# dusk-network/dusk-blindbidproof

Hardware: AMD Instinct MI355X
Metric: blind-bid proofs/sec (higher is better)
Workload: dtype u32

## Files before the change

### dusk_blindbidproof_amd/csrc/msm.hip

```cpp
#include "context.h"

namespace bbp {

#ifndef BBP_FOLD_PRIO
#define BBP_FOLD_PRIO 2
#endif
#ifndef BBP_MSM_WAVES
#define BBP_MSM_WAVES 2
#endif
#ifndef BBP_MSM_WAVES_MAX
#define BBP_MSM_WAVES_MAX 2
#endif

#ifdef BBP_MSM_PROF
__device__ unsigned long long g_msm_prof[8];
#define MSM_PROF_BEGIN() unsigned long long prof_t = wall_clock64()
#define MSM_PROF_MARK(i)                                                    \
    if (tid == 0) {                                                         \
        unsigned long long now_ = wall_clock64();                           \
        atomicAdd(&g_msm_prof[i], now_ - prof_t);                           \
        prof_t = now_;                                                      \
    }
#else
#define MSM_PROF_BEGIN()
#define MSM_PROF_MARK(i)
#endif

__device__ __forceinline__ ge ge_shfl_down(const ge& p, int d) {
    ge r;
    const u32* w = reinterpret_cast<const u32*>(&p);
    u32* o = reinterpret_cast<u32*>(&r);
#pragma unroll
    for (int i = 0; i < GE_WORDS; i++) o[i] = (u32)__shfl_down((int)w[i], d, 64);
    return r;
}

__device__ __forceinline__ void xch_put(u32* xch, const ge& p) {
    const u32* w = reinterpret_cast<const u32*>(&p);
#pragma unroll
    for (int i = 0; i < GE_WORDS; i++) xch[i] = w[i];
}

__device__ __forceinline__ ge xch_get(const u32* xch) {
    ge p;
    u32* w = reinterpret_cast<u32*>(&p);
#pragma unroll
    for (int i = 0; i < GE_WORDS; i++) w[i] = xch[i];
    return p;
}

__device__ __forceinline__ row_regs load_row(const niels_row* __restrict__ tab, u32 entry, u32* __restrict__ fault) {
    u32 row = entry & 0x7fffffffu;
    if (row > (u32)(TAB_BASES * MSM_POS - 1)) {
        row = (u32)(TAB_BASES * MSM_POS - 1);
        atomicOr(fault, 1u);
    }
#ifdef BBP_EXP_ROWMASK
    row &= BBP_EXP_ROWMASK;
#endif
    return load_row_at(tab + row, entry >> 31);
}

#ifdef BBP_ACC_COOP
constexpr int COOP_IMG = 64 * 128;
__device__ __forceinline__ u32 coop_clamp_row(u32 entry, u32* __restrict__ fault) {
    u32 row = entry & 0x7fffffffu;
    if (row > (u32)(TAB_BASES * MSM_POS - 1)) {
        row = (u32)(TAB_BASES * MSM_POS - 1);
        atomicOr(fault, 1u);
    }
    return row;
}
__device__ __forceinline__ void coop_issue(const niels_row* __restrict__ tab, u8* wb, u32 my_row, int lane, u32 srcoff) {
    const u8* t = reinterpret_cast<const u8*>(tab);
    u32 r[8];
#pragma unroll
    for (int j = 0; j < 8; j++) r[j] = (u32)__shfl((int)my_row, 8 * j + (lane >> 3), 64);
#pragma unroll
    for (int j = 0; j < 8; j++) {
        const u8* src = t + (size_t)r[j] * 128 + (srcoff ^ (u32)((j & 1) << 6));
        __builtin_amdgcn_global_load_lds((const __attribute__((address_space(1))) void*)src, (__attribute__((address_space(3))) void*)(wb + j * 1024), 16, 0, 0);
    }
}
__device__ __forceinline__ row_regs coop_read(const u8* wb, u32 A, u32 neg) {
    const u32 An = A ^ (neg << 6);
    const uint4 a0 = *reinterpret_cast<const uint4*>(wb + An), a1 = *reinterpret_cast<const uint4*>(wb + (An ^ 0x10u));
    const uint2 a2 = *reinterpret_cast<const uint2*>(wb + (An ^ 0x20u));
    const uint4 b0 = *reinterpret_cast<const uint4*>(wb + (An ^ 0x40u)), b1 = *reinterpret_cast<const uint4*>(wb + (An ^ 0x50u));
    const uint2 b2 = *reinterpret_cast<const uint2*>(wb + (An ^ 0x60u));
    const uint2 x0 = *reinterpret_cast<const uint2*>(wb + (A ^ 0x20u) + 8);
    const uint4 x1 = *reinterpret_cast<const uint4*>(wb + (A ^ 0x30u));
    const uint2 x2 = *reinterpret_cast<const uint2*>(wb + (A ^ 0x60u) + 8), x3 = *reinterpret_cast<const uint2*>(wb + (A ^ 0x70u));
    row_regs r;
    r.ypx = fe{{(i32)a0.x, (i32)a0.y, (i32)a0.z, (i32)a0.w, (i32)a1.x, (i32)a1.y, (i32)a1.z, (i32)a1.w, (i32)a2.x, (i32)a2.y}};
    r.ymx = fe{{(i32)b0.x, (i32)b0.y, (i32)b0.z, (i32)b0.w, (i32)b1.x, (i32)b1.y, (i32)b1.z, (i32)b1.w, (i32)b2.x, (i32)b2.y}};
    r.xy2d = fe{{(i32)x0.x, (i32)x0.y, (i32)x1.x, (i32)x1.y, (i32)x1.z, (i32)x1.w, (i32)x2.x, (i32)x2.y, (i32)x3.x, (i32)x3.y}};
    return r;
}
#endif

__device__ __noinline__ void ge_add_nc(ge& r, const ge& a, const ge& b) { r = ge_add(a, b); }
__device__ __noinline__ void ge_dbl_nc(ge& r, const ge& a) { r = ge_dbl(a); }

#ifndef BBP_SORT_T
#define BBP_SORT_T 1024
#endif
constexpr int SORT_T = BBP_SORT_T;
template <int MODE> struct msm_geom;
template <> struct msm_geom<0> { static constexpr int K = MSM_K, NAF = MSM_NAF, W = MSM_W; };
template <> struct msm_geom<1> { static constexpr int K = FOLD_K, NAF = FOLD_NAF, W = FOLD_W; };
template <> struct msm_geom<2> { static constexpr int K = SMALL_K, NAF = SMALL_NAF, W = SMALL_W; };

template <int MODE>
__global__ __launch_bounds__(SORT_T) void k_msm_sort(const u32* __restrict__ scal_a, const u32* __restrict__ aux, u32 n_total, u32 n_idx_sets,
                                                      u32 n_sub, u32 split, u32* __restrict__ sorted_all, u32* __restrict__ cursor_all,
                                                      const u32* __restrict__ msm_map, const u32* __restrict__ n_active, u32* __restrict__ ticket) {
    constexpr int K = msm_geom<MODE>::K, NAF = msm_geom<MODE>::NAF, W = msm_geom<MODE>::W, G = K >= SORT_T ? K / SORT_T : 1;
    __shared__ u32 cursor[K + 1];
    __shared__ u32 part[SORT_T];
    const int tid = threadIdx.x;
    if (ticket && blockIdx.x == 0 && tid == 0) *ticket = 0;
    if (n_active && blockIdx.x >= *n_active) return;
    const size_t work = blockIdx.x, msm = work / split;
    const u32 i0 = (u32)(work % split) * n_sub;
    const u32 n = i0 < n_total ? min(n_sub, n_total - i0) : 0u;
    __builtin_amdgcn_s_setprio(3);
    const u32* sbase;
    const u32* base_idx = nullptr;
    u32 base0 = 0;
    if (MODE != 1) {
        const size_t src = msm_map ? (size_t)msm_map[msm] : msm;
        sbase = scal_a + (src * (size_t)n_total + i0) * 8;
        base_idx = aux + (size_t)(msm % n_idx_sets) * n_total + i0;
    } else {
        const u32 side = (u32)msm & 1u;
        sbase = (side ? aux : scal_a) + ((msm >> 1) * (size_t)2048 + i0) * 8;
        base0 = (side ? BBP_BASE_H0 : BBP_BASE_G0) + i0;
    }
    u32* sorted = sorted_all + work * (size_t)n_sub * W;
    auto key = [&](u32 i, u32 mag) -> u32 { return (MODE != 1 ? 0u : ((i0 + i) & (FOLD_CLS - 1)) * FOLD_M) + ((mag + 1) >> 1); };

    for (int k = tid; k <= K; k += SORT_T) cursor[k] = 0;
    __syncthreads();
    for (u32 i = tid; i < n; i += SORT_T) {
        const uint4* sp = reinterpret_cast<const uint4*>(sbase + (size_t)i * 8);
        uint4 lo = sp[0], hi = sp[1];
        const u32 s[8] = {lo.x, lo.y, lo.z, lo.w, hi.x, hi.y, hi.z, hi.w};
        if (MODE != 1 && base_idx[i] == MSM_SKIP_BASE) continue;
        sc_for_each_naf_digit<NAF>(s, [&](u32, u32 mag, u32) { atomicAdd(&cursor[key(i, mag)], 1u); });
    }
    __syncthreads();
    {
        u32 local = 0;
        for (int r = 1; r <= G; r++)
            if (tid * G + r <= K) local += cursor[tid * G + r];
        const int lane = tid & 63, wave = tid >> 6;
        u32 incl = local;
#pragma unroll
        for (int d = 1; d < 64; d <<= 1) {
            const u32 up = (u32)__shfl_up((int)incl, d, 64);
            if (lane >= d) incl += up;
        }
        if (lane == 63) part[wave] = incl;
        __syncthreads();
        if (tid < 64) {
            constexpr int NW = SORT_T / 64;
            u32 v = tid < NW ? part[tid] : 0u, sc_ = v;
#pragma unroll
            for (int d = 1; d < 64; d <<= 1) {
                const u32 up = (u32)__shfl_up((int)sc_, d, 64);
                if (tid >= d) sc_ += up;
            }
            if (tid < NW) part[tid] = sc_ - v;
        }
        __syncthreads();
        u32 base = part[wave] + incl - local;
        for (int r = 1; r <= G; r++) {
            if (tid * G + r > K) break;
            const u32 c = cursor[tid * G + r];
            cursor[tid * G + r] = base;
            base += c;
        }
    }
    __syncthreads();
    for (u32 i = tid; i < n; i += SORT_T) {
        const uint4* sp = reinterpret_cast<const uint4*>(sbase + (size_t)i * 8);
        uint4 lo = sp[0], hi = sp[1];
        const u32 s[8] = {lo.x, lo.y, lo.z, lo.w, hi.x, hi.y, hi.z, hi.w};
        if (MODE != 1 && base_idx[i] == MSM_SKIP_BASE) continue;
        const u32 tb = (MODE != 1 ? base_idx[i] : base0 + i) * MSM_POS;
        sc_for_each_naf_digit<NAF>(s, [&](u32 pos, u32 mag, u32 neg) {
            u32 at = atomicAdd(&cursor[key(i, mag)], 1u);
            sorted[at] = (tb + pos) | (neg << 31);
        });
    }
    __syncthreads();
    u32* cur_out = cursor_all + work * (size_t)(K + 1);
    for (int k = tid; k <= K; k += SORT_T) cur_out[k] = k ? cursor[k] : 0u;
}

template <int MODE> struct sort_cap { static constexpr u32 V = BBP_SORT_CAP; };
template <> struct sort_cap<1> { static constexpr u32 V = 8192; };

template <int MODE>
__global__ __launch_bounds__(SORT_T) void k_msm_sort_staged(const u32* __restrict__ scal_a, const u32* __restrict__ aux, u32 n_total, u32 n_idx_sets,
                                                             u32 n_sub, u32 split, u32* __restrict__ sorted_all, u32* __restrict__ cursor_all,
                                                             const u32* __restrict__ msm_map, const u32* __restrict__ n_active, u32 CAP, u32* __restrict__ ticket) {
    constexpr int K = msm_geom<MODE>::K, NAF = msm_geom<MODE>::NAF, W = msm_geom<MODE>::W, G = K >= SORT_T ? K / SORT_T : 1;
    extern __shared__ u32 stage[];
    __shared__ u32 start[K + 2];
    __shared__ u32 fill[K + 1];
    __shared__ u32 part[SORT_T];
    const int tid = threadIdx.x;
    if (ticket && blockIdx.x == 0 && tid == 0) *ticket = 0;
    if (n_active && blockIdx.x >= *n_active) return;
    const size_t work = blockIdx.x, msm = work / split;
    const u32 i0 = (u32)(work % split) * n_sub;
    const u32 n = i0 < n_total ? min(n_sub, n_total - i0) : 0u;
    __builtin_amdgcn_s_setprio(3);
    const u32* sbase;
    const u32* base_idx = nullptr;
    u32 base0 = 0;
    if (MODE != 1) {
        const size_t src = msm_map ? (size_t)msm_map[msm] : msm;
        sbase = scal_a + (src * (size_t)n_total + i0) * 8;
        base_idx = aux + (size_t)(msm % n_idx_sets) * n_total + i0;
    } else {
        const u32 side = (u32)msm & 1u;
        sbase = (side ? aux : scal_a) + ((msm >> 1) * (size_t)2048 + i0) * 8;
        base0 = (side ? BBP_BASE_H0 : BBP_BASE_G0) + i0;
    }
    u32* sorted = sorted_all + work * (size_t)n_sub * W;
    auto key = [&](u32 i, u32 mag) -> u32 { return (MODE != 1 ? 0u : ((i0 + i) & (FOLD_CLS - 1)) * FOLD_M) + ((mag + 1) >> 1); };

    for (int k = tid; k <= K; k += SORT_T) fill[k] = 0;
    __syncthreads();
    for (u32 i = tid; i < n; i += SORT_T) {
        const uint4* sp = reinterpret_cast<const uint4*>(sbase + (size_t)i * 8);
        uint4 lo = sp[0], hi = sp[1];
        const u32 s[8] = {lo.x, lo.y, lo.z, lo.w, hi.x, hi.y, hi.z, hi.w};
        if (MODE != 1 && base_idx[i] == MSM_SKIP_BASE) continue;
        sc_for_each_naf_digit<NAF>(s, [&](u32, u32 mag, u32) { atomicAdd(&fill[key(i, mag)], 1u); });
    }
    __syncthreads();
    {
        u32 local = 0;
        for (int r = 1; r <= G; r++)
            if (tid * G + r <= K) local += fill[tid * G + r];
        const int lane = tid & 63, wave = tid >> 6;
        u32 incl = local;
#pragma unroll
        for (int d = 1; d < 64; d <<= 1) {
            const u32 up = (u32)__shfl_up((int)incl, d, 64);
            if (lane >= d) incl += up;
        }
        if (lane == 63) part[wave] = incl;
        __syncthreads();
        if (tid < 64) {
            constexpr int NW = SORT_T / 64;
            u32 v = tid < NW ? part[tid] : 0u, sc_ = v;
#pragma unroll
            for (int d = 1; d < 64; d <<= 1) {
                const u32 up = (u32)__shfl_up((int)sc_, d, 64);
                if (tid >= d) sc_ += up;
            }
            if (tid < NW) part[tid] = sc_ - v;
        }
        __syncthreads();
        u32 base = part[wave] + incl - local;
        for (int r = 1; r <= G; r++) {
            if (tid * G + r > K) break;
            const u32 c = fill[tid * G + r];
            start[tid * G + r] = base;
            fill[tid * G + r] = 0;
            base += c;
        }
        if (tid == SORT_T - 1) start[K + 1] = base;
        if (tid == 0) start[0] = 0;
    }
    __syncthreads();
    u32 kb = 1;
    while (kb <= (u32)K) {
        const u32 base = start[kb];
        const bool direct = start[kb + 1] - base > CAP;
        u32 ke = kb + 1;
        if (!direct) {
            u32 lo = kb + 1, hi = (u32)K + 1;
            while (lo < hi) {
                const u32 mid = (lo + hi + 1) >> 1;
                if (start[mid] - base <= CAP) lo = mid; else hi = mid - 1;
            }
            ke = lo;
        }
        if (start[ke] != base) {
            for (u32 i = tid; i < n; i += SORT_T) {
                const uint4* sp = reinterpret_cast<const uint4*>(sbase + (size_t)i * 8);
                uint4 lo4 = sp[0], hi4 = sp[1];
                const u32 s[8] = {lo4.x, lo4.y, lo4.z, lo4.w, hi4.x, hi4.y, hi4.z, hi4.w};
                if (MODE != 1 && base_idx[i] == MSM_SKIP_BASE) continue;
                const u32 tb = (MODE != 1 ? base_idx[i] : base0 + i) * MSM_POS;
                sc_for_each_naf_digit<NAF>(s, [&](u32 pos, u32 mag, u32 neg) {
                    const u32 k = key(i, mag);
                    if (k >= kb && k < ke) {
                        const u32 at = start[k] + atomicAdd(&fill[k], 1u);
                        const u32 ent = (tb + pos) | (neg << 31);
                        if (direct) sorted[at] = ent; else stage[at - base] = ent;
                    }
                });
            }
            __syncthreads();
            if (!direct) {
                const u32 cnt = start[ke] - base;
                for (u32 i = tid; i < cnt; i += SORT_T) sorted[base + i] = stage[i];
            }
            __syncthreads();
        }
        kb = ke;
    }
    u32* cur_out = cursor_all + work * (size_t)(K + 1);
    for (int k = tid; k <= K; k += SORT_T) cur_out[k] = k ? start[k + 1] : 0u;
}

#ifndef BBP_ACC_WG
#define BBP_ACC_WG 256
#endif
constexpr int ACC_WG = BBP_ACC_WG, ACC_WGS = ACC_T / ACC_WG;
static_assert(ACC_T % ACC_WG == 0 && ACC_WG % 64 == 0, "accumulate workgroup geometry");

template <int MODE>
__global__ __launch_bounds__(ACC_WG) __attribute__((amdgpu_waves_per_eu(BBP_MSM_WAVES, BBP_MSM_WAVES_MAX)))
void k_msm_acc(const niels_row* __restrict__ ptable, const u32* __restrict__ sorted_all, const u32* __restrict__ cursor_all, u32 n ,
               ge* __restrict__ bsum_all, ge* __restrict__ psum_all, ge* __restrict__ out, const u32* __restrict__ n_active, u32* __restrict__ fault,
               u32 n_work, u32* __restrict__ ticket) {
    constexpr int K = msm_geom<MODE>::K, W = msm_geom<MODE>::W, G = K / MSM_T;
    __shared__ u32 cursor[K + 1];
#ifdef BBP_ACC_PERSIST
    static_assert(ACC_WGS == 1, "the persistent form draws whole MSMs");
    __shared__ u32 s_ticket;
  for (;;) {
    __syncthreads();
    if (threadIdx.x == 0) s_ticket = atomicAdd(ticket, 1u);
    __syncthreads();
    const size_t msm = s_ticket;
    if (msm >= n_work || (n_active && msm >= *n_active)) return;
    const int tid = (int)threadIdx.x;
#else
    const size_t msm = blockIdx.x / ACC_WGS;
    const int tid = (int)(blockIdx.x % ACC_WGS) * ACC_WG + (int)threadIdx.x;
    if (n_active && msm >= *n_active) return;
#endif
    const u32* sorted = sorted_all + msm * (size_t)n * W;
#ifdef BBP_MSM_PRIO
    __builtin_amdgcn_s_setprio(BBP_MSM_PRIO);
#endif
    MSM_PROF_BEGIN();
    {
        const u32* cur_in = cursor_all + msm * (size_t)(K + 1);
        for (int k = threadIdx.x; k <= K; k += ACC_WG) cursor[k] = cur_in[k];
    }
    __syncthreads();
    MSM_PROF_MARK(1);

    const u32 E = cursor[K];
    ge* bsum = bsum_all + msm * (size_t)K;
    ge* psum = psum_all + msm * (size_t)ACC_T;
#ifdef BBP_KO_ACC_PERMILLE
    const u32 c0 = (u32)(((u64)tid * E) / ACC_T), c1 = c0 + (u32)(((u64)((u32)(((u64)(tid + 1) * E) / ACC_T) - c0) * BBP_KO_ACC_PERMILLE) / 1000);
#else
    const u32 c0 = (u32)(((u64)tid * E) / ACC_T), c1 = (u32)(((u64)(tid + 1) * E) / ACC_T);
#endif
#ifdef BBP_MSM_PROF
    const unsigned long long clk0 = clock64();
#endif
    u32 k_first = 0;
    bool inside = false;
#ifdef BBP_ACC_COOP
    {
        __shared__ __attribute__((aligned(1024))) u8 rowimg[ACC_WG / 64][COOP_IMG];
        const int lane = (int)threadIdx.x & 63;
        u8* wb = rowimg[threadIdx.x >> 6];
        const u32 A = (u32)lane * 128u + ((((u32)lane >> 1) & 7u) << 4);
        const u32 srcoff = (((u32)lane & 7u) ^ (((u32)lane >> 3) >> 1)) << 4;
        const u32 n_it = (E + (u32)ACC_T - 1) / (u32)ACC_T, len = c1 - c0;
        u32 k = 1, kend = 0;
        ge* dest = &psum[tid];
        if (len) {
            u32 lo = 1, hi = K;
            while (lo < hi) {
                u32 mid = (lo + hi) >> 1;
                if (cursor[mid] > c0) hi = mid; else lo = mid + 1;
            }
            k = lo, kend = cursor[k];
            k_first = lo;
            inside = cursor[k - 1] < c0;
            if (!inside) dest = &bsum[k - 1];
        }
        ge acc = ge_identity();
        u32 ent_cur = len ? sorted[c0] : 0u;
        u32 ent_nxt = len > 1 ? sorted[c0 + 1] : 0u;
        if (n_it) coop_issue(ptable, wb, coop_clamp_row(ent_cur, fault), lane, srcoff);
        for (u32 it = 0; it < n_it; it++) {
            const u32 e = c0 + it;
            const row_regs cur = coop_read(wb, A, ent_cur >> 31);
            const bool neg = ent_cur >> 31;
            ent_cur = ent_nxt;
            const bool live = it < len;
            if (live && e == kend) {
                *dest = acc;
                acc = ge_identity();
                do { k++; kend = cursor[k]; } while (kend == e);
                dest = &bsum[k - 1];
            }
            asm volatile("s_waitcnt lgkmcnt(0)" ::: "memory");
            if (it + 1 < n_it) coop_issue(ptable, wb, coop_clamp_row(ent_cur, fault), lane, srcoff);
            if (it + 2 < len) ent_nxt = sorted[e + 2]; else ent_nxt = 0u;
            if (live) acc = ge_madd_row(acc, cur, neg);
        }
        if (len) *dest = acc;
    }
#else
    if (c0 < c1) {
        u32 lo = 1, hi = K;
        while (lo < hi) {
            u32 mid = (lo + hi) >> 1;
            if (cursor[mid] > c0) hi = mid; else lo = mid + 1;
        }
        u32 k = lo, kend = cursor[k];
        k_first = lo;
        inside = cursor[k - 1] < c0;
        ge* dest = inside ? &psum[tid] : &bsum[k - 1];
        ge acc = ge_identity();
        u32 ent_cur = sorted[c0];
        u32 ent_nxt = (c0 + 1 < c1) ? sorted[c0 + 1] : 0u;
        row_regs row = load_row(ptable, ent_cur, fault);
        for (u32 e = c0; e < c1; e++) {
            if (e == kend) {
                *dest = acc;
                acc = ge_identity();
                do { k++; kend = cursor[k]; } while (kend == e);
                dest = &bsum[k - 1];
            }
            const row_regs cur = row;
            const bool neg = ent_cur >> 31;
            ent_cur = ent_nxt;
            if (e + 1 < c1) row = load_row(ptable, ent_cur, fault);
            if (e + 2 < c1) ent_nxt = sorted[e + 2];
            acc = ge_madd_row(acc, cur, neg);
        }
        *dest = acc;
    }
#endif
#ifdef BBP_MSM_PROF
    if (tid == 0) atomicAdd(&g_msm_prof[6], clock64() - clk0);
#endif
    MSM_PROF_MARK(2);
    __threadfence_block();
    __syncthreads();
    MSM_PROF_MARK(3);
#ifdef BBP_ACC_PERSIST
  }
#endif
}

template <int MODE>
__global__ __launch_bounds__(MSM_T) void k_msm_fold(const u32* __restrict__ cursor_all, ge* __restrict__ bsum_all, const ge* __restrict__ psum_all,
                                                     ge* __restrict__ out, const u32* __restrict__ n_active) {
    constexpr int K = msm_geom<MODE>::K, G = K / MSM_T;
    __shared__ u32 cursor[K + 1];
    __shared__ u32 xch[GE_WORDS];
    const int tid = threadIdx.x;
    if (n_active && blockIdx.x >= *n_active) return;
    __builtin_amdgcn_s_setprio(BBP_FOLD_PRIO);
    const size_t msm = blockIdx.x;
    {
        const u32* cur_in = cursor_all + msm * (size_t)(K + 1);
        for (int k = tid; k <= K; k += MSM_T) cursor[k] = cur_in[k];
    }
    __syncthreads();
    const u32 E = cursor[K];
    ge* bsum = bsum_all + msm * (size_t)K;
    const ge* psum = psum_all + msm * (size_t)ACC_T;
#ifdef BBP_KO_FOLD
    if (MODE != 1) { if (tid == 0) out[msm] = bsum[0]; }
    else if (tid < FOLD_CLS) out[msm * FOLD_CLS + tid] = bsum[tid];
    return;
#endif
    for (u32 ch = tid; ch < (u32)ACC_T; ch += MSM_T) {
        const u32 c0 = (u32)(((u64)ch * E) / ACC_T), c1 = (u32)(((u64)(ch + 1) * E) / ACC_T);
        if (c0 >= c1) continue;
        u32 lo = 1, hi = K;
        while (lo < hi) {
            u32 mid = (lo + hi) >> 1;
            if (cursor[mid] > c0) hi = mid; else lo = mid + 1;
        }
        const u32 k_first = lo;
        const bool inside = cursor[lo - 1] < c0;
        const bool last_of_run = inside && !(c1 < E && c1 > cursor[k_first - 1] && c1 < cursor[k_first]);
        if (last_of_run) {
            ge part = psum[ch];
            for (int u = (int)ch - 1; u >= 0; u--) {
                const u32 cu = (u32)(((u64)u * E) / ACC_T), cu1 = (u32)(((u64)(u + 1) * E) / ACC_T);
                if (cu <= cursor[k_first - 1]) break;
                if (cu1 > cu) ge_add_nc(part, part, psum[u]);
            }
            ge head = bsum[k_first - 1];
            ge_add_nc(head, head, part);
            bsum[k_first - 1] = head;
        }
    }
    __threadfence_block();
    __syncthreads();

    ge running = ge_identity(), total = ge_identity();
    if constexpr (G == 1) {
        if (cursor[tid + 1] != cursor[tid]) running = bsum[tid];
        total = running;
    } else {
#pragma unroll 1
        for (int r = G; r >= 1; r--) {
            const u32 k = tid * G + r;
            if (cursor[k] != cursor[k - 1]) running = ge_add(running, bsum[k - 1]);
            total = ge_add(total, running);
        }
    }

    if constexpr (MODE != 1) {
        const int lane = tid & 63, wave = tid >> 6;
#pragma unroll 1
        for (int d = 1; d < 64; d <<= 1) {
            ge other = ge_shfl_down(running, d);
            if (lane + d < 64) running = ge_add(running, other);
        }
        if (MSM_T > 64) {
            if (tid == 64) xch_put(xch, running);
            __syncthreads();
            if (wave == 0) {
                ge other = xch_get(xch);
                ge_add_nc(running, running, other);
            }
        }
        ge x = total;
        if (tid >= 1) {
            ge s = running;
            constexpr int LOG_G = G == 1 ? 0 : G == 2 ? 1 : G == 4 ? 2 : G == 8 ? 3 : G == 16 ? 4 : -1;
            static_assert(LOG_G >= 0, "buckets per fold lane must be a power of two up to 16");
            for (int i = 0; i < LOG_G; i++) ge_dbl_nc(s, s);
            ge_add_nc(x, x, s);
        }
#pragma unroll 1
        for (int d = 32; d >= 1; d >>= 1) {
            ge other = ge_shfl_down(x, d);
            if (lane < d) x = ge_add(x, other);
        }
        if (MSM_T > 64) {
            __syncthreads();
            if (tid == 64) xch_put(xch, x);
            __syncthreads();
        }
        if (tid == 0) {
            if (MSM_T > 64) {
                ge other = xch_get(xch);
                ge_add_nc(x, x, other);
            }
            ge other;
            ge_dbl_nc(x, x);
            other = ge_neg(running);
            ge_add_nc(x, x, other);
            out[msm] = x;
        }
    } else {
        constexpr int LPC = FOLD_M / G, LOG_G2 = G == 32 ? 5 : 6;
        static_assert(G == 32 || G == 64, "class reduction written for 4 or 2 lanes per class");
        const int q = tid & (LPC - 1);
        ge suf = running;
        for (int d = 1; d < LPC; d++) {
            ge other = ge_shfl_down(running, d);
            if (q + d < LPC) ge_add_nc(suf, suf, other);
        }
        ge x = total;
        if (q >= 1) {
            ge sg = suf;
            for (int i = 0; i < LOG_G2; i++) ge_dbl_nc(sg, sg);
            ge_add_nc(x, x, sg);
        }
        ge accq = x;
        for (int d = 1; d < LPC; d++) {
            ge other = ge_shfl_down(x, d);
            if (q == 0) ge_add_nc(accq, accq, other);
        }
        if (q == 0) {
            ge_dbl_nc(accq, accq);
            ge other = ge_neg(suf);
            ge_add_nc(accq, accq, other);
            out[msm * FOLD_CLS + (tid / LPC)] = accq;
        }
    }
}

constexpr int FOLD2_L = 32;
constexpr int FOLD2_G = MSM_K / FOLD2_L;
constexpr int FOLD2_LOG_G = 5;
static_assert(FOLD2_G == 32 && ACC_T % FOLD2_L == 0, "fold geometry");

__device__ __forceinline__ ge ge_shfl_down32(const ge& p, int d) {
    ge r;
    const u32* w = reinterpret_cast<const u32*>(&p);
    u32* o = reinterpret_cast<u32*>(&r);
#pragma unroll
    for (int i = 0; i < GE_WORDS; i++) o[i] = (u32)__shfl_down((int)w[i], d, 32);
    return r;
}

__device__ __forceinline__ ge ge_add_t2d(const ge& p, const fe& p2d, const ge& q) {
    fe a = fe_mul(fe_sub(p.Y, p.X), fe_sub(q.Y, q.X));
    fe b = fe_mul(fe_add(p.Y, p.X), fe_add(q.Y, q.X));
    fe c = fe_mul(p2d, q.T);
    fe zz = fe_mul(p.Z, q.Z);
    fe d = fe_add(zz, zz);
    fe e = fe_sub(b, a), f = fe_sub(d, c), g = fe_add(d, c), h = fe_add(b, a);
    ge r;
    r.X = fe_mul(e, f);
    r.Y = fe_mul(g, h);
    r.Z = fe_mul(g, f);
    r.T = fe_mul(e, h);
    return r;
}

__device__ __forceinline__ void park_put(u32* park, int tid, const ge& p) {
    const u32* w = reinterpret_cast<const u32*>(&p);
#pragma unroll
    for (int i = 0; i < GE_WORDS; i++) park[i * 64 + tid] = w[i];
}

__device__ __forceinline__ ge park_get(const u32* park, int tid) {
    ge p;
    u32* w = reinterpret_cast<u32*>(&p);
#pragma unroll
    for (int i = 0; i < GE_WORDS; i++) w[i] = park[i * 64 + tid];
    return p;
}

__device__ __forceinline__ ge ld_ge(const ge* p) {
    ge r;
    const uint4* s = reinterpret_cast<const uint4*>(p);
    u32* o = reinterpret_cast<u32*>(&r);
#pragma unroll
    for (int i = 0; i < GE_WORDS / 4; i++) {
        const uint4 v = s[i];
        o[4 * i] = v.x, o[4 * i + 1] = v.y, o[4 * i + 2] = v.z, o[4 * i + 3] = v.w;
    }
    return r;
}

#ifndef BBP_FOLD_WAVES
#define BBP_FOLD_WAVES 2
#endif
__global__ __launch_bounds__(64) __attribute__((amdgpu_waves_per_eu(BBP_FOLD_WAVES, BBP_FOLD_WAVES))) void k_msm_fold_half(const u32* __restrict__ cursor_all, ge* __restrict__ bsum_all, const ge* __restrict__ psum_all,
                                                       ge* __restrict__ out, u32 n_work, const u32* __restrict__ n_active) {
    constexpr int K = MSM_K, G = FOLD2_G;
    __shared__ u32 cursor2[2][K + 1];
    __shared__ u32 park[GE_WORDS * 64];
    const int tid = threadIdx.x, half = tid >> 5, l = tid & 31;
    const u32 n_tot = n_active ? min(*n_active, n_work) : n_work;
    if (2u * blockIdx.x >= n_tot) return;
    __builtin_amdgcn_s_setprio(BBP_FOLD_PRIO);
    const size_t msm = 2 * (size_t)blockIdx.x + half;
    const bool valid = msm < n_tot;
    u32* cursor = cursor2[half];
    {
        const u32* cur_in = cursor_all + msm * (size_t)(K + 1);
        for (int k = l; k <= K; k += FOLD2_L) cursor[k] = valid ? cur_in[k] : 0u;
    }
    __syncthreads();
    const u32 E = cursor[K];
    ge* bsum = bsum_all + (valid ? msm : 0) * (size_t)K;
    const ge* psum = psum_all + (valid ? msm : 0) * (size_t)ACC_T;
#pragma unroll 1
    for (u32 ch = l; ch < (u32)ACC_T; ch += FOLD2_L) {
        const u32 c0 = (u32)(((u64)ch * E) / ACC_T), c1 = (u32)(((u64)(ch + 1) * E) / ACC_T);
        bool last_of_run = false;
        u32 k_first = 1;
        if (c0 < c1) {
            u32 lo = 1, hi = K;
            while (lo < hi) {
                u32 mid = (lo + hi) >> 1;
                if (cursor[mid] > c0) hi = mid; else lo = mid + 1;
            }
            k_first = lo;
            const bool inside = cursor[lo - 1] < c0;
            last_of_run = inside && !(c1 < E && c1 > cursor[k_first - 1] && c1 < cursor[k_first]);
        }
        if (last_of_run) {
            ge part = ld_ge(&psum[ch]);
            for (int u = (int)ch - 1; u >= 0; u--) {
                const u32 cu = (u32)(((u64)u * E) / ACC_T), cu1 = (u32)(((u64)(u + 1) * E) / ACC_T);
                if (cu <= cursor[k_first - 1]) break;
                if (cu1 > cu) {
                    const ge more = ld_ge(&psum[u]);
                    part = ge_add(part, more);
                }
            }
            const ge head = ld_ge(&bsum[k_first - 1]);
            bsum[k_first - 1] = ge_add(head, part);
        }
    }
    __threadfence_block();
    __syncthreads();

    ge running = ge_identity();
    fe r2d = fe_zero();
    park_put(park, tid, ge_identity());
#pragma unroll 1
    for (int r = G; r >= 1; r--) {
        const u32 k = (u32)l * G + r;
        if (cursor[k] != cursor[k - 1]) {
            const ge cur = ld_ge(&bsum[k - 1]);
            running = ge_add_t2d(running, r2d, cur);
            r2d = fe_mul(running.T, fe_d2());
        }
        const ge total = park_get(park, tid);
        park_put(park, tid, ge_add_t2d(running, r2d, total));
    }

    ge v = running;
#pragma unroll 1
    for (int it = 0; it < 12; it++) {
        ge q;
        bool take;
        int n_dbl = 0;
        if (it == 5) {
            q = v;
            v = park_get(park, tid);
            park_put(park, tid, q);
            n_dbl = FOLD2_LOG_G;
            take = l >= 1;
        } else if (it == 11) {
            q = ge_neg(park_get(park, tid));
            take = true;
        } else {
            const int d = it < 5 ? (1 << it) : (16 >> (it - 6));
            q = ge_shfl_down32(v, d);
            take = it < 5 ? (l + d < 32) : (l < d);
        }
        if (it == 11) {
            v = ge_dbl(v);
        } else {
#pragma unroll 1
            for (int i = 0; i < n_dbl; i++) q = ge_dbl(q);
        }
        if (take) v = ge_add(v, q);
    }
    if (l == 0 && valid) out[msm] = v;
}

constexpr int REDUCE_L = 16;
__global__ __launch_bounds__(64) void k_msm_reduce(u32 n_out, u32 split, u32 items, const ge* __restrict__ tmp, ge* __restrict__ out) {
    __builtin_amdgcn_s_setprio(3);
    const u32 t = blockIdx.x * blockDim.x + threadIdx.x;
    const u32 o = t / REDUCE_L, j = t % REDUCE_L;
    const u32 msm = o / items, c = o % items;
    ge acc = ge_identity();
    if (o < n_out && j < split) acc = tmp[((size_t)msm * split + j) * items + c];
    for (u32 jj = j + REDUCE_L; o < n_out && jj < split; jj += REDUCE_L)
        acc = ge_add(acc, tmp[((size_t)msm * split + jj) * items + c]);
#pragma unroll 1
    for (int d = REDUCE_L / 2; d >= 1; d >>= 1) {
        const ge other = ge_shfl_down(acc, d);
        if ((int)j < d) acc = ge_add(acc, other);
    }
    if (o < n_out && j == 0) out[o] = acc;
}


struct MsmScratch {
    u32 *sorted, *cursor;
    ge *bsum, *psum, *tmp;
    u32* ticket;
    size_t bytes;
};
static MsmScratch msm_scratch_layout(void* base, size_t n_msm, size_t n_terms, size_t W, size_t K, size_t out_items = 1) {
    auto up = [](size_t x) { return (x + 255) / 256 * 256; };
    MsmScratch m;
    size_t o = 0;
    m.sorted = reinterpret_cast<u32*>(static_cast<u8*>(base) + o);
    o += up(n_msm * n_terms * W * sizeof(u32));
    m.cursor = reinterpret_cast<u32*>(static_cast<u8*>(base) + o);
    o += up(n_msm * (K + 1) * sizeof(u32));
    m.bsum = reinterpret_cast<ge*>(static_cast<u8*>(base) + o);
    o += n_msm * K * sizeof(ge);
    m.psum = reinterpret_cast<ge*>(static_cast<u8*>(base) + o);
    o += n_msm * ACC_T * sizeof(ge);
    m.tmp = reinterpret_cast<ge*>(static_cast<u8*>(base) + o);
    o += up(n_msm * out_items * sizeof(ge));
    m.ticket = reinterpret_cast<u32*>(static_cast<u8*>(base) + o);
    o += 256;
    m.bytes = o;
    return m;
}
size_t msm_scratch_bytes(uint32_t n_msm, uint32_t n_terms) {
    const u32 split = msm_split(n_msm, n_terms), n_sub = (n_terms + split - 1) / split;
    size_t a = msm_scratch_layout(nullptr, (size_t)n_msm * split, n_sub, MSM_W, MSM_K).bytes;
    if (split > 1) a = std::max(a, msm_scratch_layout(nullptr, (size_t)n_msm * split, n_sub, SMALL_W, SMALL_K).bytes);
    const size_t b = msm_scratch_layout(nullptr, n_msm, n_terms, MSM_W, MSM_K).bytes;
    return a > b ? a : b;
}

static inline u32 acc_grid(bbp_ctx*, u32 n_work) {
#ifdef BBP_ACC_PERSIST
    static const u32 cap = [] { const char* e = getenv("BBP_ACC_PERSIST_GRID"); return e ? (u32)atoi(e) : 512u; }();
    return n_work < cap ? n_work : cap;
#else
    return n_work * ACC_WGS;
#endif
}

int32_t fold_generators_launch(bbp_ctx* ctx, uint32_t n_proofs, const sc* g_dev, const sc* h_dev, ge* out_dev, hipStream_t stream,
                               int scratch_slot) {
    if (n_proofs == 0) return BBP_OK;
    const size_t n_msm = 2 * (size_t)n_proofs;
    const u32 split = msm_split((u32)n_msm, 2048), n_sub = (2048 + split - 1) / split;
    const size_t n_work = n_msm * split;
    DevBuf& scratch = ctx->slice_fold[scratch_slot];
    int32_t rc = dev_reserve(ctx, scratch, msm_scratch_layout(nullptr, n_work, n_sub, FOLD_W, FOLD_K, FOLD_CLS).bytes);
    if (rc) return rc;
    const MsmScratch m = msm_scratch_layout(scratch.p, n_work, n_sub, FOLD_W, FOLD_K, FOLD_CLS);
    {
        ScopedEvent ev(ctx, TAG_MSM_SORT, stream);
        if (ctx->msm_knobs.sort_staged & 2) {
            if (!ctx->sort_lds_attr1) {
                BBP_HIP_TRY(ctx, hipFuncSetAttribute((const void*)k_msm_sort_staged<1>, hipFuncAttributeMaxDynamicSharedMemorySize, (int)(sort_cap<1>::V * 4)));
                ctx->sort_lds_attr1 = true;
            }
            hipLaunchKernelGGL(k_msm_sort_staged<1>, dim3((u32)n_work), dim3(SORT_T), sort_cap<1>::V * 4, stream, (const u32*)g_dev, (const u32*)h_dev, 2048u, 1u,
                               n_sub, split, m.sorted, m.cursor, (const u32*)nullptr, (const u32*)nullptr, sort_cap<1>::V, m.ticket);
        } else
            hipLaunchKernelGGL(k_msm_sort<1>, dim3((u32)n_work), dim3(SORT_T), 0, stream, (const u32*)g_dev, (const u32*)h_dev, 2048u, 1u, n_sub, split,
                               m.sorted, m.cursor, (const u32*)nullptr, (const u32*)nullptr, m.ticket);
        BBP_HIP_TRY(ctx, hipGetLastError());
    }
    {
        ScopedEvent ev(ctx, TAG_MSM, stream);
        hipLaunchKernelGGL(k_msm_acc<1>, dim3(acc_grid(ctx, (u32)n_work)), dim3(ACC_WG), 0, stream, ctx->ptable, m.sorted, m.cursor, n_sub, m.bsum, m.psum,
                           split > 1 ? m.tmp : out_dev, (const u32*)nullptr, ctx->health, (u32)n_work, m.ticket);
        BBP_HIP_TRY(ctx, hipGetLastError());
    }
    ScopedEvent evf(ctx, TAG_MSM_FOLD, stream);
    hipLaunchKernelGGL(k_msm_fold<1>, dim3((u32)n_work), dim3(MSM_T), 0, stream, m.cursor, m.bsum, m.psum, split > 1 ? m.tmp : out_dev,
                       (const u32*)nullptr);
    BBP_HIP_TRY(ctx, hipGetLastError());
    if (split > 1) {
        const u32 n_out = (u32)n_msm * FOLD_CLS;
        hipLaunchKernelGGL(k_msm_reduce, dim3((n_out * REDUCE_L + 63) / 64), dim3(64), lds_token(ctx), stream, n_out, split, (u32)FOLD_CLS, m.tmp, out_dev);
        BBP_HIP_TRY(ctx, hipGetLastError());
    }
    return BBP_OK;
}

__global__ __launch_bounds__(64) void k_encode(const ge* __restrict__ pts, u32 n, u32* __restrict__ out_words) {
    u32 i = blockIdx.x * blockDim.x + threadIdx.x;
    if (i >= n) return;
    ge p = pts[i];
    u32 w[8];
    ge_encode_words(w, p);
    uint4* o = reinterpret_cast<uint4*>(out_words + (size_t)i * 8);
    o[0] = make_uint4(w[0], w[1], w[2], w[3]);
    o[1] = make_uint4(w[4], w[5], w[6], w[7]);
}

__global__ void k_debug_poke(u32* sorted) { sorted[0] = 0x7ffffff0u; }

int32_t msm_launch(bbp_ctx* ctx, uint32_t n_msm, uint32_t n_terms, const u32* scalars_dev, const u32* base_idx_dev,
                   ge* out_points_dev, hipStream_t stream, uint32_t n_idx_sets, int scratch_slot, const u32* msm_map_dev,
                   const u32* n_active_dev, bool chain_acc) {
    if (n_msm == 0) return BBP_OK;
    if (n_terms == 0 || n_terms > 65535u) {
        ctx->err = "msm_launch: n_terms out of range";
        return BBP_ERR_BAD_ARG;
    }
    DevBuf& scratch = scratch_slot ? ctx->slice_sorted[scratch_slot] : ctx->sorted;
    int32_t rc = dev_reserve(ctx, scratch, msm_scratch_bytes(n_msm, n_terms));
    if (rc) return rc;
    const MsmPlan plan = plan_msm(ctx->msm_knobs, n_msm, n_terms, n_active_dev != nullptr);
    const u32 split = plan.split, n_sub = plan.n_sub, n_work = plan.n_work;
    if (plan.geom == MsmPlan::SMALL) {
        const MsmScratch ms = msm_scratch_layout(scratch.p, n_work, n_sub, SMALL_W, SMALL_K);
        {
            ScopedEvent ev(ctx, TAG_MSM_SORT, stream);
            hipLaunchKernelGGL(k_msm_sort<2>, dim3(n_work), dim3(SORT_T), 0, stream, scalars_dev, base_idx_dev, n_terms, n_idx_sets, n_sub, split, ms.sorted, ms.cursor,
                               msm_map_dev, n_active_dev, ms.ticket);
            BBP_HIP_TRY(ctx, hipGetLastError());
        }
        if (ctx->debug_corrupt) {
            ctx->debug_corrupt = 0;
            hipLaunchKernelGGL(k_debug_poke, dim3(1), dim3(1), 0, stream, ms.sorted);
            BBP_HIP_TRY(ctx, hipGetLastError());
        }
        {
            ScopedEvent ev(ctx, TAG_MSM, stream);
            hipLaunchKernelGGL(k_msm_acc<2>, dim3(acc_grid(ctx, n_work)), dim3(ACC_WG), 0, stream, ctx->ptable, ms.sorted, ms.cursor, n_sub, ms.bsum, ms.psum, ms.tmp,
                               n_active_dev, ctx->health, n_work, ms.ticket);
            BBP_HIP_TRY(ctx, hipGetLastError());
        }
        {
            ScopedEvent evf(ctx, TAG_MSM_FOLD, stream);
            hipLaunchKernelGGL(k_msm_fold<2>, dim3(n_work), dim3(MSM_T), 0, stream, ms.cursor, ms.bsum, ms.psum, ms.tmp, n_active_dev);
            BBP_HIP_TRY(ctx, hipGetLastError());
        }
        hipLaunchKernelGGL(k_msm_reduce, dim3((n_msm * REDUCE_L + 63) / 64), dim3(64), lds_token(ctx), stream, n_msm, split, 1u, ms.tmp, out_points_dev);
        BBP_HIP_TRY(ctx, hipGetLastError());
        return BBP_OK;
    }
    const MsmScratch m = msm_scratch_layout(scratch.p, n_work, n_sub, MSM_W, MSM_K);
    {
        ScopedEvent ev(ctx, TAG_MSM_SORT, stream);
        if (plan.sort != MsmPlan::PLAIN) {
            const u32 cap = plan.sort_cap;
            if (!ctx->sort_lds_attr) {
                BBP_HIP_TRY(ctx, hipFuncSetAttribute((const void*)k_msm_sort_staged<0>, hipFuncAttributeMaxDynamicSharedMemorySize, (int)(SORT_CAP_WIDE * 4)));
                ctx->sort_lds_attr = true;
            }
            hipLaunchKernelGGL(k_msm_sort_staged<0>, dim3(n_work), dim3(SORT_T), cap * 4, stream, scalars_dev, base_idx_dev, n_terms, n_idx_sets, n_sub, split,
                               m.sorted, m.cursor, msm_map_dev, n_active_dev, cap, m.ticket);
        }
        else
            hipLaunchKernelGGL(k_msm_sort<0>, dim3(n_work), dim3(SORT_T), 0, stream, scalars_dev, base_idx_dev, n_terms, n_idx_sets, n_sub, split,
                               m.sorted, m.cursor, msm_map_dev, n_active_dev, m.ticket);
        BBP_HIP_TRY(ctx, hipGetLastError());
    }
    if (ctx->debug_corrupt) {
        ctx->debug_corrupt = 0;
        hipLaunchKernelGGL(k_debug_poke, dim3(1), dim3(1), 0, stream, m.sorted);
        BBP_HIP_TRY(ctx, hipGetLastError());
    }
    chain_acc = chain_acc && ctx->verify_serial_acc;
    if (chain_acc && ctx->vacc_valid)
        BBP_HIP_TRY(ctx, hipStreamWaitEvent(stream, ctx->ev_vacc[ctx->vacc_seq % bbp_ctx::VACC_RING], 0));
    {
        ScopedEvent ev(ctx, TAG_MSM, stream);
        hipLaunchKernelGGL(k_msm_acc<0>, dim3(acc_grid(ctx, n_work)), dim3(ACC_WG), 0, stream, ctx->ptable, m.sorted, m.cursor, n_sub, m.bsum, m.psum,
                           split > 1 ? m.tmp : out_points_dev, n_active_dev, ctx->health, n_work, m.ticket);
        BBP_HIP_TRY(ctx, hipGetLastError());
    }
    static const bool chain_after_fold = getenv("BBP_VERIFY_CHAIN_AFTER_FOLD") && atoi(getenv("BBP_VERIFY_CHAIN_AFTER_FOLD"));
    if (chain_acc && !chain_after_fold) {
        ctx->vacc_seq++;
        BBP_HIP_TRY(ctx, hipEventRecord(ctx->ev_vacc[ctx->vacc_seq % bbp_ctx::VACC_RING], stream));
        ctx->vacc_valid = true;
    }
    ScopedEvent evf(ctx, TAG_MSM_FOLD, stream);
    if (plan.fold == MsmPlan::HALF)
        hipLaunchKernelGGL(k_msm_fold_half, dim3((n_work + 1) / 2), dim3(64), 0, stream, m.cursor, m.bsum, m.psum, split > 1 ? m.tmp : out_points_dev,
                           n_work, n_active_dev);
    else
        hipLaunchKernelGGL(k_msm_fold<0>, dim3(n_work), dim3(MSM_T), 0, stream, m.cursor, m.bsum, m.psum, split > 1 ? m.tmp : out_points_dev, n_active_dev);
    BBP_HIP_TRY(ctx, hipGetLastError());
    if (chain_acc && chain_after_fold) {
        ctx->vacc_seq++;
        BBP_HIP_TRY(ctx, hipEventRecord(ctx->ev_vacc[ctx->vacc_seq % bbp_ctx::VACC_RING], stream));
        ctx->vacc_valid = true;
    }
    if (plan.reduce) {
        hipLaunchKernelGGL(k_msm_reduce, dim3((n_msm * REDUCE_L + 63) / 64), dim3(64), lds_token(ctx), stream, n_msm, split, 1u, m.tmp, out_points_dev);
        BBP_HIP_TRY(ctx, hipGetLastError());
    }
#ifdef BBP_MSM_PROF
    static int launches = 0;
    if (++launches % 16 == 0) {
        unsigned long long h[8];
        (void)hipStreamSynchronize(stream);
        (void)hipMemcpyFromSymbol(h, HIP_SYMBOL(g_msm_prof), sizeof h);
        fprintf(stderr, "[msm prof, %d launches, 10ns ticks of lane 0 summed over WGs] load %llu D1 %llu D1wait %llu D2 %llu E %llu; D1 shader clock %.0f MHz\n", launches,
                h[1], h[2], h[3], h[4], h[5], 100.0 * (double)h[6] / (double)h[2]);
    }
#endif
    return BBP_OK;
}

int32_t encode_launch(bbp_ctx* ctx, uint32_t n, const ge* pts_dev, uint8_t* out32_dev, hipStream_t stream) {
    if (n == 0) return BBP_OK;
    ScopedEvent ev(ctx, TAG_ENCODE, stream);
    hipLaunchKernelGGL(k_encode, dim3((n + 63) / 64), dim3(64), lds_token(ctx), stream, pts_dev, n, (u32*)out32_dev);
    BBP_HIP_TRY(ctx, hipGetLastError());
    return BBP_OK;
}

}
```

Baseline: 21700.

## Publish per-chunk bucket words from accumulate so fold skips cursor binary searches

The accumulate kernel now writes a compact per-chunk word (first bucket index plus an inside-run flag) to a new scratch array. The fold kernels use these words to find run ends and walk partial sums, instead of recomputing chunk bounds with divisions and binary searches over the cursor array in shared memory. The half-fold kernel drops its shared cursor copy, reads the cursor bitmask of non-empty buckets straight from global memory, and seeds the running sum from the top bucket. It also gains an optional BBP_FOLD_FIT path that interleaves bucket and park additions. The cost is an extra global write per chunk plus more scratch memory, and the backward scan now performs scattered global reads of cword.

```diff
diff --git a/dusk_blindbidproof_amd/csrc/msm.hip b/dusk_blindbidproof_amd/csrc/msm.hip
--- a/dusk_blindbidproof_amd/csrc/msm.hip
+++ b/dusk_blindbidproof_amd/csrc/msm.hip
@@ -321,6 +321,19 @@
     for (int k = tid; k <= K; k += SORT_T) cur_out[k] = k ? start[k + 1] : 0u;
 }
 
+__device__ __forceinline__ u32 chunk_word(u32 k_first, bool inside) { return k_first | ((u32)inside << 31); }
+
+__device__ __forceinline__ bool chunk_ends_run(const u32* __restrict__ cword, u32 ch, u32 K, u32& k_first) {
+    const u32 w = cword[ch];
+    k_first = w & 0x7fffffffu;
+    if (!(w >> 31) || k_first - 1u >= K) return false;
+    for (u32 nx = ch + 1; nx < (u32)ACC_T; nx++) {
+        const u32 x = cword[nx];
+        if (x) return x != w;
+    }
+    return true;
+}
+
 #ifndef BBP_ACC_WG
 #define BBP_ACC_WG 256
 #endif
@@ -330,8 +343,8 @@
 template <int MODE>
 __global__ __launch_bounds__(ACC_WG) __attribute__((amdgpu_waves_per_eu(BBP_MSM_WAVES, BBP_MSM_WAVES_MAX)))
 void k_msm_acc(const niels_row* __restrict__ ptable, const u32* __restrict__ sorted_all, const u32* __restrict__ cursor_all, u32 n ,
-               ge* __restrict__ bsum_all, ge* __restrict__ psum_all, ge* __restrict__ out, const u32* __restrict__ n_active, u32* __restrict__ fault,
-               u32 n_work, u32* __restrict__ ticket) {
+               ge* __restrict__ bsum_all, ge* __restrict__ psum_all, u32* __restrict__ cword_all, ge* __restrict__ out, const u32* __restrict__ n_active,
+               u32* __restrict__ fault, u32 n_work, u32* __restrict__ ticket) {
     constexpr int K = msm_geom<MODE>::K, W = msm_geom<MODE>::W, G = K / MSM_T;
     __shared__ u32 cursor[K + 1];
 #ifdef BBP_ACC_PERSIST
@@ -364,6 +377,7 @@
     const u32 E = cursor[K];
     ge* bsum = bsum_all + msm * (size_t)K;
     ge* psum = psum_all + msm * (size_t)ACC_T;
+    u32* cword = cword_all + msm * (size_t)ACC_T;
 #ifdef BBP_KO_ACC_PERMILLE
     const u32 c0 = (u32)(((u64)tid * E) / ACC_T), c1 = c0 + (u32)(((u64)((u32)(((u64)(tid + 1) * E) / ACC_T) - c0) * BBP_KO_ACC_PERMILLE) / 1000);
 #else
@@ -395,6 +409,7 @@
             inside = cursor[k - 1] < c0;
             if (!inside) dest = &bsum[k - 1];
         }
+        cword[tid] = len ? chunk_word(k_first, inside) : 0u;
         ge acc = ge_identity();
         u32 ent_cur = len ? sorted[c0] : 0u;
         u32 ent_nxt = len > 1 ? sorted[c0 + 1] : 0u;
@@ -428,6 +443,7 @@
         u32 k = lo, kend = cursor[k];
         k_first = lo;
         inside = cursor[k - 1] < c0;
+        cword[tid] = chunk_word(k_first, inside);
         ge* dest = inside ? &psum[tid] : &bsum[k - 1];
         ge acc = ge_identity();
         u32 ent_cur = sorted[c0];
@@ -448,7 +464,8 @@
             acc = ge_madd_row(acc, cur, neg);
         }
         *dest = acc;
-    }
+    } else
+        cword[tid] = 0u;
 #endif
 #ifdef BBP_MSM_PROF
     if (tid == 0) atomicAdd(&g_msm_prof[6], clock64() - clk0);
@@ -464,7 +481,7 @@
 
 template <int MODE>
 __global__ __launch_bounds__(MSM_T) void k_msm_fold(const u32* __restrict__ cursor_all, ge* __restrict__ bsum_all, const ge* __restrict__ psum_all,
-                                                     ge* __restrict__ out, const u32* __restrict__ n_active) {
+                                                     const u32* __restrict__ cword_all, ge* __restrict__ out, const u32* __restrict__ n_active) {
     constexpr int K = msm_geom<MODE>::K, G = K / MSM_T;
     __shared__ u32 cursor[K + 1];
     __shared__ u32 xch[GE_WORDS];
@@ -477,36 +494,28 @@
         for (int k = tid; k <= K; k += MSM_T) cursor[k] = cur_in[k];
     }
     __syncthreads();
-    const u32 E = cursor[K];
     ge* bsum = bsum_all + msm * (size_t)K;
     const ge* psum = psum_all + msm * (size_t)ACC_T;
+    const u32* cword = cword_all + msm * (size_t)ACC_T;
 #ifdef BBP_KO_FOLD
     if (MODE != 1) { if (tid == 0) out[msm] = bsum[0]; }
     else if (tid < FOLD_CLS) out[msm * FOLD_CLS + tid] = bsum[tid];
     return;
 #endif
     for (u32 ch = tid; ch < (u32)ACC_T; ch += MSM_T) {
-        const u32 c0 = (u32)(((u64)ch * E) / ACC_T), c1 = (u32)(((u64)(ch + 1) * E) / ACC_T);
-        if (c0 >= c1) continue;
-        u32 lo = 1, hi = K;
-        while (lo < hi) {
-            u32 mid = (lo + hi) >> 1;
-            if (cursor[mid] > c0) hi = mid; else lo = mid + 1;
-        }
-        const u32 k_first = lo;
-        const bool inside = cursor[lo - 1] < c0;
-        const bool last_of_run = inside && !(c1 < E && c1 > cursor[k_first - 1] && c1 < cursor[k_first]);
-        if (last_of_run) {
-            ge part = psum[ch];
-            for (int u = (int)ch - 1; u >= 0; u--) {
-                const u32 cu = (u32)(((u64)u * E) / ACC_T), cu1 = (u32)(((u64)(u + 1) * E) / ACC_T);
-                if (cu <= cursor[k_first - 1]) break;
-                if (cu1 > cu) ge_add_nc(part, part, psum[u]);
-            }
-            ge head = bsum[k_first - 1];
-            ge_add_nc(head, head, part);
-            bsum[k_first - 1] = head;
-        }
+        u32 k_first;
+        if (!chunk_ends_run(cword, ch, K, k_first)) continue;
+        const u32 mine = chunk_word(k_first, true);
+        ge part = psum[ch];
+        for (int u = (int)ch - 1; u >= 0; u--) {
+            const u32 x = cword[u];
+            if (!x) continue;
+            if (x != mine) break;
+            ge_add_nc(part, part, psum[u]);
+        }
+        ge head = bsum[k_first - 1];
+        ge_add_nc(head, head, part);
+        bsum[k_first - 1] = head;
     }
     __threadfence_block();
     __syncthreads();
@@ -656,65 +665,122 @@
 #define BBP_FOLD_WAVES 2
 #endif
 __global__ __launch_bounds__(64) __attribute__((amdgpu_waves_per_eu(BBP_FOLD_WAVES, BBP_FOLD_WAVES))) void k_msm_fold_half(const u32* __restrict__ cursor_all, ge* __restrict__ bsum_all, const ge* __restrict__ psum_all,
-                                                       ge* __restrict__ out, u32 n_work, const u32* __restrict__ n_active) {
+                                                       const u32* __restrict__ cword_all, ge* __restrict__ out, u32 n_work, const u32* __restrict__ n_active) {
     constexpr int K = MSM_K, G = FOLD2_G;
-    __shared__ u32 cursor2[2][K + 1];
     __shared__ u32 park[GE_WORDS * 64];
+#ifdef BBP_FOLD_FIT
+    __shared__ u32 s_slot[2][GE_WORDS];
+#endif
     const int tid = threadIdx.x, half = tid >> 5, l = tid & 31;
     const u32 n_tot = n_active ? min(*n_active, n_work) : n_work;
     if (2u * blockIdx.x >= n_tot) return;
     __builtin_amdgcn_s_setprio(BBP_FOLD_PRIO);
     const size_t msm = 2 * (size_t)blockIdx.x + half;
     const bool valid = msm < n_tot;
-    u32* cursor = cursor2[half];
-    {
-        const u32* cur_in = cursor_all + msm * (size_t)(K + 1);
-        for (int k = l; k <= K; k += FOLD2_L) cursor[k] = valid ? cur_in[k] : 0u;
-    }
-    __syncthreads();
-    const u32 E = cursor[K];
     ge* bsum = bsum_all + (valid ? msm : 0) * (size_t)K;
     const ge* psum = psum_all + (valid ? msm : 0) * (size_t)ACC_T;
+    const u32* cword = cword_all + (valid ? msm : 0) * (size_t)ACC_T;
+    u32 full = 0;
+    if (valid) {
+        const u32* cur = cursor_all + msm * (size_t)(K + 1) + (size_t)l * G;
+        u32 prev = cur[0];
+#pragma unroll
+        for (int r = 1; r <= G; r++) {
+            const u32 c = cur[r];
+            full |= (u32)(c != prev) << (r - 1);
+            prev = c;
+        }
+    }
 #pragma unroll 1
     for (u32 ch = l; ch < (u32)ACC_T; ch += FOLD2_L) {
-        const u32 c0 = (u32)(((u64)ch * E) / ACC_T), c1 = (u32)(((u64)(ch + 1) * E) / ACC_T);
-        bool last_of_run = false;
-        u32 k_first = 1;
-        if (c0 < c1) {
-            u32 lo = 1, hi = K;
-            while (lo < hi) {
-                u32 mid = (lo + hi) >> 1;
-                if (cursor[mid] > c0) hi = mid; else lo = mid + 1;
-            }
-            k_first = lo;
-            const bool inside = cursor[lo - 1] < c0;
-            last_of_run = inside && !(c1 < E && c1 > cursor[k_first - 1] && c1 < cursor[k_first]);
-        }
-        if (last_of_run) {
+        u32 k_first;
+        if (valid && chunk_ends_run(cword, ch, K, k_first)) {
+            const u32 mine = chunk_word(k_first, true);
             ge part = ld_ge(&psum[ch]);
-            for (int u = (int)ch - 1; u >= 0; u--) {
-                const u32 cu = (u32)(((u64)u * E) / ACC_T), cu1 = (u32)(((u64)(u + 1) * E) / ACC_T);
-                if (cu <= cursor[k_first - 1]) break;
-                if (cu1 > cu) {
-                    const ge more = ld_ge(&psum[u]);
-                    part = ge_add(part, more);
+            int u = (int)ch - 1;
+            bool head = false;
+#pragma unroll 1
+            while (!head) {
+                const ge* src = &bsum[k_first - 1];
+                head = true;
+                for (; u >= 0; u--) {
+                    const u32 x = cword[u];
+                    if (!x) continue;
+                    if (x == mine) {
+                        src = &psum[u--];
+                        head = false;
+                    }
+                    break;
                 }
-            }
-            const ge head = ld_ge(&bsum[k_first - 1]);
-            bsum[k_first - 1] = ge_add(head, part);
+                const ge q = ld_ge(src);
+                part = ge_add(part, q);
+            }
+            bsum[k_first - 1] = part;
         }
     }
     __threadfence_block();
     __syncthreads();
 
     ge running = ge_identity();
-    fe r2d = fe_zero();
-    park_put(park, tid, ge_identity());
-#pragma unroll 1
-    for (int r = G; r >= 1; r--) {
-        const u32 k = (u32)l * G + r;
-        if (cursor[k] != cursor[k - 1]) {
-            const ge cur = ld_ge(&bsum[k - 1]);
+    if (full >> (G - 1)) running = ld_ge(&bsum[l * G + G - 1]);
+    fe r2d = fe_mul(running.T, fe_d2());
+    park_put(park, tid, running);
+#ifdef BBP_FOLD_FIT
+#pragma unroll 1
+    for (int j = 2; j < 2 * G; j++) {
+        const int r = G - (j >> 1);
+        const bool bucket = !(j & 1);
+        bool act = true;
+        ge q;
+        if (bucket) {
+            act = (full >> (r - 1)) & 1u;
+            q = ld_ge(&bsum[l * G + (act ? r - 1 : 0)]);
+        } else
+            q = park_get(park, tid);
+        if (act) {
+            const ge sum = ge_add_t2d(running, r2d, q);
+            if (bucket) {
+                running = sum;
+                r2d = fe_mul(sum.T, fe_d2());
+            } else
+                park_put(park, tid, sum);
+        }
+    }
+
+    ge v = running;
+#pragma unroll 1
+    for (int it = 0; it < 12; it++) {
+        int n_dbl = 0;
+        if (it == 5) {
+            if (l == 0) {
+                xch_put(s_slot[half], v);
+                v = ge_identity();
+            }
+            n_dbl = FOLD2_LOG_G;
+        } else if (it == 11)
+            n_dbl = 1;
+#pragma unroll 1
+        for (int i = 0; i < n_dbl; i++) v = ge_dbl(v);
+        ge q;
+        bool take;
+        if (it == 5) {
+            q = park_get(park, tid);
+            take = true;
+        } else if (it == 11) {
+            q = ge_neg(xch_get(s_slot[half]));
+            take = l == 0;
+        } else {
+            const int d = it < 5 ? (1 << it) : (16 >> (it - 6));
+            q = ge_shfl_down32(v, d);
+            take = it < 5 ? (l + d < 32) : (l < d);
+        }
+        if (take) v = ge_add(v, q);
+    }
+#else
+#pragma unroll 1
+    for (int r = G - 1; r >= 1; r--) {
+        if ((full >> (r - 1)) & 1u) {
+            const ge cur = ld_ge(&bsum[l * G + r - 1]);
             running = ge_add_t2d(running, r2d, cur);
             r2d = fe_mul(running.T, fe_d2());
         }
@@ -750,6 +816,7 @@
         }
         if (take) v = ge_add(v, q);
     }
+#endif
     if (l == 0 && valid) out[msm] = v;
 }
 
@@ -775,6 +842,7 @@
 struct MsmScratch {
     u32 *sorted, *cursor;
     ge *bsum, *psum, *tmp;
+    u32* cword;
     u32* ticket;
     size_t bytes;
 };
@@ -790,6 +858,8 @@
     o += n_msm * K * sizeof(ge);
     m.psum = reinterpret_cast<ge*>(static_cast<u8*>(base) + o);
     o += n_msm * ACC_T * sizeof(ge);
+    m.cword = reinterpret_cast<u32*>(static_cast<u8*>(base) + o);
+    o += up(n_msm * ACC_T * sizeof(u32));
     m.tmp = reinterpret_cast<ge*>(static_cast<u8*>(base) + o);
     o += up(n_msm * out_items * sizeof(ge));
     m.ticket = reinterpret_cast<u32*>(static_cast<u8*>(base) + o);
@@ -840,12 +910,12 @@
     }
     {
         ScopedEvent ev(ctx, TAG_MSM, stream);
-        hipLaunchKernelGGL(k_msm_acc<1>, dim3(acc_grid(ctx, (u32)n_work)), dim3(ACC_WG), 0, stream, ctx->ptable, m.sorted, m.cursor, n_sub, m.bsum, m.psum,
+        hipLaunchKernelGGL(k_msm_acc<1>, dim3(acc_grid(ctx, (u32)n_work)), dim3(ACC_WG), 0, stream, ctx->ptable, m.sorted, m.cursor, n_sub, m.bsum, m.psum, m.cword,
                            split > 1 ? m.tmp : out_dev, (const u32*)nullptr, ctx->health, (u32)n_work, m.ticket);
         BBP_HIP_TRY(ctx, hipGetLastError());
     }
     ScopedEvent evf(ctx, TAG_MSM_FOLD, stream);
-    hipLaunchKernelGGL(k_msm_fold<1>, dim3((u32)n_work), dim3(MSM_T), 0, stream, m.cursor, m.bsum, m.psum, split > 1 ? m.tmp : out_dev,
+    hipLaunchKernelGGL(k_msm_fold<1>, dim3((u32)n_work), dim3(MSM_T), 0, stream, m.cursor, m.bsum, m.psum, m.cword, split > 1 ? m.tmp : out_dev,
                        (const u32*)nullptr);
     BBP_HIP_TRY(ctx, hipGetLastError());
     if (split > 1) {
@@ -897,13 +967,13 @@
         }
         {
             ScopedEvent ev(ctx, TAG_MSM, stream);
-            hipLaunchKernelGGL(k_msm_acc<2>, dim3(acc_grid(ctx, n_work)), dim3(ACC_WG), 0, stream, ctx->ptable, ms.sorted, ms.cursor, n_sub, ms.bsum, ms.psum, ms.tmp,
+            hipLaunchKernelGGL(k_msm_acc<2>, dim3(acc_grid(ctx, n_work)), dim3(ACC_WG), 0, stream, ctx->ptable, ms.sorted, ms.cursor, n_sub, ms.bsum, ms.psum, ms.cword, ms.tmp,
                                n_active_dev, ctx->health, n_work, ms.ticket);
             BBP_HIP_TRY(ctx, hipGetLastError());
         }
         {
             ScopedEvent evf(ctx, TAG_MSM_FOLD, stream);
-            hipLaunchKernelGGL(k_msm_fold<2>, dim3(n_work), dim3(MSM_T), 0, stream, ms.cursor, ms.bsum, ms.psum, ms.tmp, n_active_dev);
+            hipLaunchKernelGGL(k_msm_fold<2>, dim3(n_work), dim3(MSM_T), 0, stream, ms.cursor, ms.bsum, ms.psum, ms.cword, ms.tmp, n_active_dev);
             BBP_HIP_TRY(ctx, hipGetLastError());
         }
         hipLaunchKernelGGL(k_msm_reduce, dim3((n_msm * REDUCE_L + 63) / 64), dim3(64), lds_token(ctx), stream, n_msm, split, 1u, ms.tmp, out_points_dev);
@@ -937,7 +1007,7 @@
         BBP_HIP_TRY(ctx, hipStreamWaitEvent(stream, ctx->ev_vacc[ctx->vacc_seq % bbp_ctx::VACC_RING], 0));
     {
         ScopedEvent ev(ctx, TAG_MSM, stream);
-        hipLaunchKernelGGL(k_msm_acc<0>, dim3(acc_grid(ctx, n_work)), dim3(ACC_WG), 0, stream, ctx->ptable, m.sorted, m.cursor, n_sub, m.bsum, m.psum,
+        hipLaunchKernelGGL(k_msm_acc<0>, dim3(acc_grid(ctx, n_work)), dim3(ACC_WG), 0, stream, ctx->ptable, m.sorted, m.cursor, n_sub, m.bsum, m.psum, m.cword,
                            split > 1 ? m.tmp : out_points_dev, n_active_dev, ctx->health, n_work, m.ticket);
         BBP_HIP_TRY(ctx, hipGetLastError());
     }
@@ -949,10 +1019,10 @@
     }
     ScopedEvent evf(ctx, TAG_MSM_FOLD, stream);
     if (plan.fold == MsmPlan::HALF)
-        hipLaunchKernelGGL(k_msm_fold_half, dim3((n_work + 1) / 2), dim3(64), 0, stream, m.cursor, m.bsum, m.psum, split > 1 ? m.tmp : out_points_dev,
+        hipLaunchKernelGGL(k_msm_fold_half, dim3((n_work + 1) / 2), dim3(64), 0, stream, m.cursor, m.bsum, m.psum, m.cword, split > 1 ? m.tmp : out_points_dev,
                            n_work, n_active_dev);
     else
-        hipLaunchKernelGGL(k_msm_fold<0>, dim3(n_work), dim3(MSM_T), 0, stream, m.cursor, m.bsum, m.psum, split > 1 ? m.tmp : out_points_dev, n_active_dev);
+        hipLaunchKernelGGL(k_msm_fold<0>, dim3(n_work), dim3(MSM_T), 0, stream, m.cursor, m.bsum, m.psum, m.cword, split > 1 ? m.tmp : out_points_dev, n_active_dev);
     BBP_HIP_TRY(ctx, hipGetLastError());
     if (chain_acc && chain_after_fold) {
         ctx->vacc_seq++;
```

Result: no change. 21770 (median of 4 runs) (+0.3%).
